# semicolonTransistor/rust-ray-tracing

Measured on AMD Instinct MI355X. Metric: Msamples/s (pixels×spp/s), 1920×1080·512spp·500 spheres; 1/2/4/8 GPU, higher is better.
Workload: dtype f32

## Files before the change

rust-ray-tracing_amd/csrc/rt_sweep.hpp:

```cpp
#pragma once
#include "rt_common.hpp"

namespace rt {

__device__ __forceinline__ uint32_t filter_group(const SphGroup<float>& cur, f2 K0, f2 K1, f2 K2, f2 K3, uint32_t& s0,
                                                 uint32_t& s1, f2* D = nullptr) {
    const f2 cx0 = {cur.v[0], cur.v[1]}, cy0 = {cur.v[2], cur.v[3]}, cz0 = {cur.v[4], cur.v[5]}, rr0 = {cur.v[6], cur.v[7]};
    const f2 cx1 = {cur.v[8], cur.v[9]}, cy1 = {cur.v[10], cur.v[11]}, cz1 = {cur.v[12], cur.v[13]}, rr1 = {cur.v[14], cur.v[15]};
    f2 a0, b0, a1, b1, r0, r1;
    asm volatile(
        "v_pk_fma_f32 %[a0], %[cz0], %[K0], %[K3] op_sel:[0,1,0] op_sel_hi:[1,1,0]\n\t"
        "v_pk_fma_f32 %[b0], %[cz0], %[K2], %[K3] op_sel:[0,0,1] op_sel_hi:[1,0,1]\n\t"
        "v_pk_fma_f32 %[a1], %[cz1], %[K0], %[K3] op_sel:[0,1,0] op_sel_hi:[1,1,0]\n\t"
        "v_pk_fma_f32 %[b1], %[cz1], %[K2], %[K3] op_sel:[0,0,1] op_sel_hi:[1,0,1]\n\t"
        "v_pk_fma_f32 %[a0], %[cx0], %[K0], %[a0] op_sel_hi:[1,0,1]\n\t"
        "v_pk_fma_f32 %[b0], %[cy0], %[K1], %[b0] op_sel:[0,1,0] op_sel_hi:[1,1,1]\n\t"
        "v_pk_fma_f32 %[a1], %[cx1], %[K0], %[a1] op_sel_hi:[1,0,1]\n\t"
        "v_pk_fma_f32 %[b1], %[cy1], %[K1], %[b1] op_sel:[0,1,0] op_sel_hi:[1,1,1]\n\t"
        "v_pk_fma_f32 %[b0], %[cx0], %[K1], %[b0] op_sel_hi:[1,0,1]\n\t"
        "v_pk_fma_f32 %[b1], %[cx1], %[K1], %[b1] op_sel_hi:[1,0,1]\n\t"
        "v_pk_fma_f32 %[r0], %[b0], %[b0], %[rr0] neg_lo:[1,0,0] neg_hi:[1,0,0]\n\t"
        "v_pk_fma_f32 %[r1], %[b1], %[b1], %[rr1] neg_lo:[1,0,0] neg_hi:[1,0,0]\n\t"
        "v_pk_fma_f32 %[r0], %[a0], %[a0], %[r0] neg_lo:[1,0,0] neg_hi:[1,0,0]\n\t"
        "v_pk_fma_f32 %[r1], %[a1], %[a1], %[r1] neg_lo:[1,0,0] neg_hi:[1,0,0]"
        : [a0] "=&v"(a0), [b0] "=&v"(b0), [a1] "=&v"(a1), [b1] "=&v"(b1), [r0] "=&v"(r0), [r1] "=&v"(r1)
        : [cx0] "s"(cx0), [cy0] "s"(cy0), [cz0] "s"(cz0), [rr0] "s"(rr0), [cx1] "s"(cx1), [cy1] "s"(cy1),
          [cz1] "s"(cz1), [rr1] "s"(rr1), [K0] "v"(K0), [K1] "v"(K1), [K2] "v"(K2), [K3] "v"(K3));
    s0 = __float_as_uint(r0.x) & __float_as_uint(r0.y);
    s1 = __float_as_uint(r1.x) & __float_as_uint(r1.y);
    if (D) { D[0] = r0; D[1] = r1; }
    return ~(s0 & s1);
}

__device__ __forceinline__ uint32_t cam_filter_group(const SphGroup<float>& cur, f2 K0, f2 K1) {
    const f2 ox0 = {cur.v[0], cur.v[1]}, oy0 = {cur.v[2], cur.v[3]}, oz0 = {cur.v[4], cur.v[5]}, sc0 = {cur.v[6], cur.v[7]};
    const f2 ox1 = {cur.v[8], cur.v[9]}, oy1 = {cur.v[10], cur.v[11]}, oz1 = {cur.v[12], cur.v[13]}, sc1 = {cur.v[14], cur.v[15]};
    f2 t0, t1;
    asm volatile(
        "v_pk_mul_f32 %[t0], %[ox0], %[K0] op_sel_hi:[1,0]\n\t"
        "v_pk_mul_f32 %[t1], %[ox1], %[K0] op_sel_hi:[1,0]\n\t"
        "v_pk_fma_f32 %[t0], %[oy0], %[K0], %[t0] op_sel:[0,1,0] op_sel_hi:[1,1,1]\n\t"
        "v_pk_fma_f32 %[t1], %[oy1], %[K0], %[t1] op_sel:[0,1,0] op_sel_hi:[1,1,1]\n\t"
        "v_pk_fma_f32 %[t0], %[oz0], %[K1], %[t0] op_sel_hi:[1,0,1]\n\t"
        "v_pk_fma_f32 %[t1], %[oz1], %[K1], %[t1] op_sel_hi:[1,0,1]\n\t"
        "v_pk_add_f32 %[t0], %[t0], %[sc0]\n\t"
        "v_pk_add_f32 %[t1], %[t1], %[sc1]"
        : [t0] "=&v"(t0), [t1] "=&v"(t1)
        : [ox0] "s"(ox0), [oy0] "s"(oy0), [oz0] "s"(oz0), [sc0] "s"(sc0), [ox1] "s"(ox1), [oy1] "s"(oy1),
          [oz1] "s"(oz1), [sc1] "s"(sc1), [K0] "v"(K0), [K1] "v"(K1));
    return (__float_as_uint(t0.x) | __float_as_uint(t0.y) | __float_as_uint(t1.x)) | __float_as_uint(t1.y);
}

__device__ __forceinline__ uint32_t box_pair(const float* v, f2 B0, f2 B1, f2 B2, f2 B3, f2 B4, float bt) {
    f2 ux, uy, uz, nx, ny, nz;
    const f2 cx = {v[0], v[1]}, cy = {v[2], v[3]}, cz = {v[4], v[5]}, hx = {v[6], v[7]}, hy = {v[8], v[9]},
             hz = {v[10], v[11]};
    asm volatile(
        "v_pk_fma_f32 %[ux], %[cx], %[B0], %[B2] op_sel_hi:[1,0,0]\n\t"
        "v_pk_fma_f32 %[uy], %[cy], %[B0], %[B2] op_sel:[0,1,1] op_sel_hi:[1,1,1]\n\t"
        "v_pk_fma_f32 %[uz], %[cz], %[B1], %[B1] op_sel:[0,0,1] op_sel_hi:[1,0,1]\n\t"
        "v_pk_fma_f32 %[nx], %[hx], %[B3], %[ux] op_sel_hi:[1,0,1] neg_lo:[0,1,0] neg_hi:[0,1,0]\n\t"
        "v_pk_fma_f32 %[ny], %[hy], %[B3], %[uy] op_sel:[0,1,0] op_sel_hi:[1,1,1] neg_lo:[0,1,0] neg_hi:[0,1,0]\n\t"
        "v_pk_fma_f32 %[nz], %[hz], %[B4], %[uz] op_sel_hi:[1,0,1] neg_lo:[0,1,0] neg_hi:[0,1,0]\n\t"
        "v_pk_fma_f32 %[ux], %[hx], %[B3], %[ux] op_sel_hi:[1,0,1]\n\t"
        "v_pk_fma_f32 %[uy], %[hy], %[B3], %[uy] op_sel:[0,1,0] op_sel_hi:[1,1,1]\n\t"
        "v_pk_fma_f32 %[uz], %[hz], %[B4], %[uz] op_sel_hi:[1,0,1]"
        : [ux] "=&v"(ux), [uy] "=&v"(uy), [uz] "=&v"(uz), [nx] "=&v"(nx), [ny] "=&v"(ny), [nz] "=&v"(nz)
        : [cx] "s"(cx), [cy] "s"(cy), [cz] "s"(cz), [hx] "s"(hx), [hy] "s"(hy), [hz] "s"(hz), [B0] "v"(B0),
          [B1] "v"(B1), [B2] "v"(B2), [B3] "v"(B3), [B4] "v"(B4));
    auto pass = [bt](float nx, float ny, float nz, float fx, float fy, float fz, auto bitc) -> uint32_t {
        constexpr uint32_t bit = decltype(bitc)::value;
        float tn, tf;
        unsigned long long m;
        uint32_t r;
        asm volatile(
            "v_max3_f32 %[tn], %[nx], %[ny], %[nz]\n\t"
            "v_min3_f32 %[tf], %[fx], %[fy], %[fz]\n\t"
            "v_max_f32 %[tn], 0, %[tn]\n\t"
            "v_min_f32 %[tf], %[tf], %[bt]\n\t"
            "v_cmp_nlt_f32_e64 %[m], %[tf], %[tn]\n\t"
            "s_cmp_lg_u64 %[m], 0\n\t"
            "s_cselect_b32 %[r], %[bit], 0"
            : [tn] "=&v"(tn), [tf] "=&v"(tf), [m] "=&s"(m), [r] "=s"(r)
            : [nx] "v"(nx), [ny] "v"(ny), [nz] "v"(nz), [fx] "v"(fx), [fy] "v"(fy), [fz] "v"(fz), [bt] "v"(bt),
              [bit] "n"(bit)
            : "scc");
        return r;
    };
    return __builtin_amdgcn_readfirstlane(pass(nx.x, ny.x, nz.x, ux.x, uy.x, uz.x, std::integral_constant<uint32_t, 1>{}) |
                                          pass(nx.y, ny.y, nz.y, ux.y, uy.y, uz.y, std::integral_constant<uint32_t, 2>{}));
}
__device__ __forceinline__ uint32_t box_mask(const BoxGroup& cur, f2 B0, f2 B1, f2 B2, f2 B3, f2 B4, float bt) {
    return box_pair(&cur.v[0], B0, B1, B2, B3, B4, bt) | (box_pair(&cur.v[12], B0, B1, B2, B3, B4, bt) << 2);
}
__device__ __forceinline__ uint32_t box_mask(const LBoxGroup& cur, f2 B0, f2 B1, f2 B2, f2 B3, f2 B4, float bt) {
    return box_pair(&cur.v[0], B0, B1, B2, B3, B4, bt) | (box_pair(&cur.v[12], B0, B1, B2, B3, B4, bt) << 2);
}

template <typename T> struct HitBest {
    T t = T(INFINITY);
    int i = -1;
    __device__ __forceinline__ T bt() const { return t; }
    __device__ __forceinline__ int bi() const { return i; }
    __device__ __forceinline__ void set(T r, uint32_t j) { t = r; i = (int)j; }
};
constexpr uint32_t kT001 = 0x3A83126Fu;
__device__ __forceinline__ uint64_t hit_key(float r, uint32_t j) {
    return ((uint64_t)(__float_as_uint(r) - kT001) << 32) | (uint64_t)~j;
}
template <> struct HitBest<float> {
    uint64_t k = (uint64_t)(0x7F800000u - kT001) << 32;
    __device__ __forceinline__ float bt() const { return __uint_as_float((uint32_t)(k >> 32) + kT001); }
    __device__ __forceinline__ int bi() const { return (int)~(uint32_t)k; }
    __device__ __forceinline__ void set(float r, uint32_t j) { k = hit_key(r, j); }
};
template <typename T, bool root2, bool SCALAR>
__device__ __forceinline__ void hit_update(T hb, T disc, uint32_t i, T a, T inv_a, HitBest<T>& bh) {
    if constexpr (SCALAR) {
        const T sd = sqrt(disc);
        T root = (-hb - sd) / a;
        if (!(root >= T(0.001) && root < T(INFINITY))) {
            root = (-hb + sd) / a;
            if (!(root >= T(0.001) && root < T(INFINITY))) return;
        }
        if (root < bh.bt() || (root == bh.bt() && (int)i < bh.bi())) bh.set(root, i);
        return;
    }
    const T sd = sqrt_len(disc);
    const T r1 = (-hb - sd) * inv_a;
    if constexpr (sizeof(T) == 4 && !root2) {
        const uint64_t key = hit_key(r1, i);
        bh.k = key < bh.k ? key : bh.k;
        return;
    }
    bool valid = r1 >= T(0.001) && r1 < T(INFINITY);
    T root = r1;
    if (root2 && !valid) {
        root = (-hb + sd) * inv_a;
        valid = root >= T(0.001) && root < T(INFINITY);
    }
    if constexpr (sizeof(T) == 4) {
        const uint64_t key = hit_key(root, i);
        const bool take = valid & (key < bh.k);
        bh.k = take ? key : bh.k;
    } else {
        const bool take = valid & ((root < bh.t) | ((root == bh.t) & ((int)i > bh.i)));
        bh.t = take ? root : bh.t;
        bh.i = take ? (int)i : bh.i;
    }
}

template <typename T, bool root2, bool SCALAR = false, bool CAMT = false, bool MEGA = false>
__device__ __forceinline__ int nearest_hit(const KParams<T>& p, const V3<T>& o, const V3<T>& d, T& t_out) {
    const T a = SCALAR ? len2(d) : pk_len2(d);
    const T inv_a = SCALAR ? T(0) : T(1.0) / a;
    HitBest<T> bh;
    KSTAT(CAMT ? 3 : 1);
    auto hit = [&](T hb, T disc, uint32_t i) { hit_update<T, root2, SCALAR>(hb, disc, i, a, inv_a, bh); };
    auto sbits = [](T x) -> uint32_t {
        if constexpr (sizeof(T) == 4) return __float_as_uint(x);
        else return (uint32_t)__double2hiint(x);
    };
    constexpr bool kBothRoots = root2 || SCALAR;
    auto is_cand = [](uint32_t m) -> bool { return (int32_t)m < 0; };
    auto cand_f = [&](T hb, T disc) -> bool { return kBothRoots ? disc >= T(0.0) : (disc >= T(0.0) && hb <= T(0.0)); };
    if constexpr (CAMT && !kBothRoots) {
        const auto& qa = *cold_args<T>();
        cptr<float> ff = (cptr<float>)__builtin_assume_aligned(qa.camf, 64);
        cptr<T> fe = (cptr<T>)__builtin_assume_aligned(qa.camsph, 64);
        const uint32_t ngf = qa.n_fgroups;
        const float fdx = (float)d.x, fdy = (float)d.y, fdz = (float)d.z;
        const float inv = 1.0f / sqrtf(__builtin_fmaf(fdz, fdz, __builtin_fmaf(fdy, fdy, fdx * fdx)));
        const f2 K0 = {fdx * inv, fdy * inv}, K1 = {fdz * inv, 0.0f};
        auto exact4 = [&](uint32_t g) {
            KSTAT(2);
            if constexpr (sizeof(T) == 4) {
                const SphGroup<T> cur = load_group(fe, g);
                const f2 dx = {d.x, d.x}, dy = {d.y, d.y}, dz = {d.z, d.z};
                const f2 na = {-a, -a};
                f2 hb[2], disc[2];
#pragma unroll
                for (uint32_t q = 0; q < 2; ++q) {
                    const T* v = &cur.v[8 * q];
                    const f2 ocx = {v[0], v[1]}, ocy = {v[2], v[3]}, ocz = {v[4], v[5]}, c = {v[6], v[7]};
                    hb[q] = fma2(ocz, dz, fma2(ocy, dy, ocx * dx));
                    disc[q] = fma2(hb[q], hb[q], na * c);
                }
                const uint32_t i0 = 4 * g;
                if (cand_f(hb[0].x, disc[0].x)) hit(hb[0].x, disc[0].x, i0);
                if (cand_f(hb[0].y, disc[0].y)) hit(hb[0].y, disc[0].y, i0 + 1);
                if (cand_f(hb[1].x, disc[1].x)) hit(hb[1].x, disc[1].x, i0 + 2);
                if (cand_f(hb[1].y, disc[1].y)) hit(hb[1].y, disc[1].y, i0 + 3);
            } else {
                const SphGroup<T> c0 = load_group(fe, 2 * g), c1 = load_group(fe, 2 * g + 1);
                T hb[4], disc[4];
#pragma unroll
                for (uint32_t j = 0; j < 4; ++j) {
                    const T* v = j < 2 ? &c0.v[4 * j] : &c1.v[4 * (j - 2)];
                    hb[j] = pk_dot(mk(v[0], v[1], v[2]), d);
                    disc[j] = fma(hb[j], hb[j], -a * v[3]);
                }
#pragma unroll
                for (uint32_t j = 0; j < 4; ++j)
                    if (cand_f(hb[j], disc[j])) hit(hb[j], disc[j], 4 * g + j);
            }
        };
        auto group = [&](const SphGroup<float>& cur, uint32_t g) {
            if (is_cand(cam_filter_group(cur, K0, K1))) exact4(g);
        };
        sphere_loop(ff, ngf, group);
    } else if constexpr (CAMT) {
        const auto& qa = *cold_args<T>();
        cptr<T> f = (cptr<T>)__builtin_assume_aligned(qa.camsph, 64);
        const uint32_t ng = qa.n_groups;
        if constexpr (sizeof(T) == 4) {
            const f2 dx = {d.x, d.x}, dy = {d.y, d.y}, dz = {d.z, d.z};
            const f2 na = {-a, -a};
            auto group = [&](const SphGroup<T>& cur, uint32_t g) {
                f2 hb[2], disc[2];
#pragma unroll
                for (uint32_t q = 0; q < 2; ++q) {
                    const T* v = &cur.v[8 * q];
                    const f2 ocx = {v[0], v[1]}, ocy = {v[2], v[3]}, ocz = {v[4], v[5]}, c = {v[6], v[7]};
                    if constexpr (SCALAR) {
                        hb[q] = (ocx * dx + ocy * dy) + ocz * dz;
                        disc[q] = hb[q] * hb[q] - (-na) * c;
                    } else {
                        hb[q] = fma2(ocz, dz, fma2(ocy, dy, ocx * dx));
                        disc[q] = fma2(hb[q], hb[q], na * c);
                    }
                }
                const uint32_t t = sbits(disc[0].x) & sbits(disc[0].y) & sbits(disc[1].x);
                const uint32_t acc = __builtin_amdgcn_bitop3_b32(t, sbits(disc[1].y), 0u, 0x3F);
                if (is_cand(acc)) {
                    KSTAT(2);
                    const uint32_t i0 = 4 * g;
                    if (cand_f(hb[0].x, disc[0].x)) hit(hb[0].x, disc[0].x, i0);
                    if (cand_f(hb[0].y, disc[0].y)) hit(hb[0].y, disc[0].y, i0 + 1);
                    if (cand_f(hb[1].x, disc[1].x)) hit(hb[1].x, disc[1].x, i0 + 2);
                    if (cand_f(hb[1].y, disc[1].y)) hit(hb[1].y, disc[1].y, i0 + 3);
                }
            };
            sphere_loop(f, ng, group);
        } else {
            auto group = [&](const SphGroup<T>& cur, uint32_t g) {
                T hb[2], disc[2];
#pragma unroll
                for (uint32_t j = 0; j < 2; ++j) {
                    const T* v = &cur.v[4 * j];
                    const V3<T> oc = mk(v[0], v[1], v[2]);
                    hb[j] = SCALAR ? dot(oc, d) : pk_dot(oc, d);
                    disc[j] = SCALAR ? hb[j] * hb[j] - a * v[3] : fma(hb[j], hb[j], -a * v[3]);
                }
                const uint32_t acc = __builtin_amdgcn_bitop3_b32(sbits(disc[0]), sbits(disc[1]), 0u, 0x3F);
                if (is_cand(acc)) {
                    KSTAT(2);
                    if (cand_f(hb[0], disc[0])) hit(hb[0], disc[0], 2 * g);
                    if (cand_f(hb[1], disc[1])) hit(hb[1], disc[1], 2 * g + 1);
                }
            };
            sphere_loop(f, ng, group);
        }
    } else {
        const auto& qa = *cold_args<T>();
        cptr<float> ff = (cptr<float>)__builtin_assume_aligned(qa.rfsph, 64);
        cptr<T> fe = (cptr<T>)__builtin_assume_aligned(qa.rsph, 64);
        auto sidx = [&](uint32_t g, cptr<float> ip) -> Q4 {
            if (ip != nullptr) {
                cptr<uint32_t> r = (cptr<uint32_t>)ip;
                return Q4{r[0], r[1], r[2], r[3]};
            }
            const auto& qi = *cold_args<T>();
            cptr<uint32_t> ri = (cptr<uint32_t>)__builtin_assume_aligned(qi.ridx, 16);
            return Q4{ri[4 * g], ri[4 * g + 1], ri[4 * g + 2], ri[4 * g + 3]};
        };
        const float fdx = (float)d.x, fdy = (float)d.y, fdz = (float)d.z;
        const float fox = (float)o.x, foy = (float)o.y, foz = (float)o.z;
        const float L = __builtin_fmaf(fdz, fdz, fdx * fdx);
        const float af = __builtin_fmaf(fdz, fdz, __builtin_fmaf(fdy, fdy, fdx * fdx));
        const float on = fabsf(fox) + fabsf(foy) + fabsf(foz);
        const float pm = qa.f_cmax + on;
        const float m = kFilterMargin * __builtin_fmaf(pm, pm, qa.f_r2max);
        const float sg = MEGA ? 1.0f : __builtin_amdgcn_rsqf(__builtin_fmaf(m, qa.f_ir2, 1.0f));
        const float s1 = __builtin_amdgcn_rsqf(L) * sg, s2 = __builtin_amdgcn_rsqf(L * af) * sg;
        float e1x = fdz * s1, e1z = -fdx * s1;
        float e2x = -(fdx * fdy) * s2, e2y = L * s2, e2z = -(fdy * fdz) * s2;
        float oe1 = __builtin_fmaf(foz, e1z, fox * e1x);
        float oe2 = __builtin_fmaf(foz, e2z, __builtin_fmaf(foy, e2y, fox * e2x));
        auto inv_ax = [](float v) -> float {
            return __builtin_amdgcn_rcpf(fabsf(v) >= 1e-20f ? v : copysignf(1e-20f, v));
        };
        float ix = inv_ax(fdx), iy = inv_ax(fdy), iz = inv_ax(fdz);
        const float kap = 1.0f + __builtin_fmaf(m, qa.f_hir2, pm * qa.f_isr);
        float Jx = fabsf(ix) * kap, Jy = fabsf(iy) * kap, Jz = fabsf(iz) * kap;
        float Ax = -(fox * ix), Ay = -(foy * iy), Az = -(foz * iz);
        if (!(L >= 1e-15f) || !(pm <= 1e15f)) {
            e1x = e1z = e2x = e2y = e2z = 0.0f;
            oe1 = oe2 = 0.0f;
            ix = iy = iz = Jx = Jy = Jz = Ax = Ay = Az = 0.0f;
        }
        const f2 K0 = {e1x, e1z}, K1 = {e2x, e2y}, K2 = {e2z, 0.0f}, K3 = {-oe1, -oe2};
        const f2 B0 = {ix, iy}, B1 = {iz, Az}, B2 = {Ax, Ay}, B3 = {Jx, Jy}, B4 = {Jz, 0.0f};
        auto btf = [&]() -> float {
            if constexpr (sizeof(T) == 4) return bh.bt();
            else return (float)bh.bt() * (1.0f + 0x1.0p-22f);
        };
        const f2 nixy = {-ix, -iy}, aixy = {fabsf(ix), fabsf(iy)};
        const float aiz = fabsf(iz);
        auto lmask = [&](const LBoxGroup& g) -> uint32_t {
            const auto& ql = *cold_args<T>();
            const f2 Sxy = {g.v[24], g.v[25]};
            const float Sz = g.v[26], Rg = g.v[27];
            f2 opxy;
            float opz;
            if constexpr (sizeof(T) == 4) {
                opxy = f2{o.x, o.y} - Sxy;
                opz = o.z - Sz;
            } else {
                opxy = f2{(float)(o.x - (double)Sxy.x), (float)(o.y - (double)Sxy.y)};
                opz = (float)(o.z - (double)Sz);
            }
            const float pmg = ((fabsf(opxy.x) + fabsf(opxy.y)) + fabsf(opz)) + Rg;
            const float kp = __builtin_fmaf(__builtin_fmaf(pmg, pmg, ql.l_r2max), ql.l_hir2,
                                            __builtin_fmaf(pmg, ql.l_isr, 1.0f));
            const f2 C1 = {iz, -(opz * iz)}, C2 = opxy * nixy;
            const f2 C3 = aixy * f2{kp, kp}, C4 = {aiz * kp, 0.0f};
            return box_mask(g, B0, C1, C2, C3, C4, btf());
        };
        auto exact4 = [&](uint32_t g, uint32_t pairs = sizeof(T) == 4 ? 3u : 15u, cptr<float> ip = nullptr) {
            KSTAT(0);
            if constexpr (sizeof(T) == 4) {
                const SphGroup<T> cur = load_group(fe, g);
                const f2 ox = {o.x, o.x}, oy = {o.y, o.y}, oz = {o.z, o.z};
                const f2 dx = {d.x, d.x}, dy = {d.y, d.y}, dz = {d.z, d.z};
                const f2 na = {-a, -a};
                const Q4 si = sidx(g, ip);
#pragma unroll
                for (uint32_t q = 0; q < 2; ++q) {
                    if (!((pairs >> q) & 1u)) continue;
                    f2 hb, disc;
                    const T* v = &cur.v[8 * q];
                    const f2 cx = {v[0], v[1]}, cy = {v[2], v[3]}, cz = {v[4], v[5]}, r2 = {v[6], v[7]};
                    const f2 ocx = ox - cx, ocy = oy - cy, ocz = oz - cz;
                    if constexpr (SCALAR) {
                        hb = (ocx * dx + ocy * dy) + ocz * dz;
                        const f2 c = ((ocx * ocx + ocy * ocy) + ocz * ocz) - r2;
                        disc = hb * hb - (-na) * c;
                    } else {
                        hb = fma2(ocz, dz, fma2(ocy, dy, ocx * dx));
                        const f2 c = fma2(ocz, ocz, fma2(ocy, ocy, ocx * ocx)) - r2;
                        disc = fma2(hb, hb, na * c);
                    }
                    if (cand_f(hb.x, disc.x)) hit(hb.x, disc.x, q ? si.z : si.x);
                    if (cand_f(hb.y, disc.y)) hit(hb.y, disc.y, q ? si.w : si.y);
                }
            } else {
                const SphGroup<T> c0 = load_group(fe, 2 * g), c1 = load_group(fe, 2 * g + 1);
                T hb[4], disc[4];
#pragma unroll
                for (uint32_t j = 0; j < 4; ++j) {
                    if (!((pairs >> j) & 1u)) continue;
                    const T* v = j < 2 ? &c0.v[4 * j] : &c1.v[4 * (j - 2)];
                    const V3<T> oc = mk(o.x - v[0], o.y - v[1], o.z - v[2]);
                    if constexpr (SCALAR) {
                        hb[j] = dot(oc, d);
                        disc[j] = hb[j] * hb[j] - a * (len2(oc) - v[3]);
                    } else {
                        hb[j] = pk_dot(oc, d);
                        const T c = pk_len2(oc) - v[3];
                        disc[j] = fma(hb[j], hb[j], -a * c);
                    }
                }
                const Q4 si = sidx(g, ip);
                const uint32_t sv[4] = {si.x, si.y, si.z, si.w};
#pragma unroll
                for (uint32_t j = 0; j < 4; ++j)
                    if (((pairs >> j) & 1u) && cand_f(hb[j], disc[j])) hit(hb[j], disc[j], sv[j]);
            }
        };
        auto exact4f = [&](const SphGroup<float>& cur, cptr<float> recp, uint32_t pairs) {
            KSTAT(0);
            if constexpr (sizeof(T) == 4) {
                cptr<uint32_t> xr = (cptr<uint32_t>)recp;
                uint32_t rec[8];
#pragma unroll
                for (int j = 0; j < 8; ++j) rec[j] = xr[(uint32_t)j];
                const f2 ox = {o.x, o.x}, oy = {o.y, o.y}, oz = {o.z, o.z};
                const f2 dx = {d.x, d.x}, dy = {d.y, d.y}, dz = {d.z, d.z};
                const f2 na = {-a, -a};
#pragma unroll
                for (uint32_t q = 0; q < 2; ++q) {
                    if (!((pairs >> q) & 1u)) continue;
                    f2 hb, disc;
                    const float* v = &cur.v[8 * q];
                    const f2 cx = {v[0], v[1]}, cy = {v[2], v[3]}, cz = {v[4], v[5]};
                    const f2 r2 = {__uint_as_float(rec[2 * q]), __uint_as_float(rec[2 * q + 1])};
                    const f2 ocx = ox - cx, ocy = oy - cy, ocz = oz - cz;
                    if constexpr (SCALAR) {
                        hb = (ocx * dx + ocy * dy) + ocz * dz;
                        const f2 c = ((ocx * ocx + ocy * ocy) + ocz * ocz) - r2;
                        disc = hb * hb - (-na) * c;
                    } else {
                        hb = fma2(ocz, dz, fma2(ocy, dy, ocx * dx));
                        const f2 c = fma2(ocz, ocz, fma2(ocy, ocy, ocx * ocx)) - r2;
                        disc = fma2(hb, hb, na * c);
                    }
                    if (cand_f(hb.x, disc.x)) hit(hb.x, disc.x, rec[4 + 2 * q]);
                    if (cand_f(hb.y, disc.y)) hit(hb.y, disc.y, rec[5 + 2 * q]);
                }
            }
        };
        const uint32_t nxg = qa.n_xg, ntop = qa.n_top;
        uint32_t n_box = 0, n_filt = 0, n_exact = 0;
        for (uint32_t g = 0; g < nxg; ++g) {
            const uint32_t pr = sizeof(T) == 4 ? (4u * g + 2u >= qa.n_xs ? 1u : 3u) : 15u;
            n_exact += pr == 1u ? 2u : 4u;
            exact4(g, pr);
        }
        cptr<float> ft = (cptr<float>)__builtin_assume_aligned(qa.ftop, 32);
        cptr<float> fs = (cptr<float>)__builtin_assume_aligned(qa.fsup, 32);
        const uint32_t nsg = (ntop + 3u) / 4u;
        auto walk_super = [&](uint32_t sup) {
            KSTAT(5);
            ++n_box;
            uint32_t mask;
            if constexpr (MEGA) {
                mask = lmask(load_lbox((cptr<float>)__builtin_assume_aligned(qa.lclb, 64), sup));
            }
            else mask = box_mask(load_box(ft, sup), B0, B1, B2, B3, B4, btf());
            while (mask != 0u) {
                const uint32_t kc = 4u * sup + (uint32_t)__builtin_ctz(mask);
                const uint32_t g0 = nxg + 4u * kc;
                mask &= mask - 1u;
                KSTAT(4);
                n_filt += 4u;
                f2 L0 = K0, L1 = K1, L2 = K2, L3 = K3;
                cptr<float> fg = ff;
                if constexpr (MEGA) {
                    const auto& ql = *cold_args<T>();
                    fg = (cptr<float>)__builtin_assume_aligned(ql.lfsph, 64) + 16u * nxg + 96u * kc;
                    const f2 Ckxy = {fg[64], fg[65]};
                    const float Ckz = fg[66];
                    const float Rc = fg[67], r2x = fg[72], ir2 = fg[73];
                    f2 opxy;
                    float opz;
                    if constexpr (sizeof(T) == 4) {
                        opxy = f2{o.x, o.y} - Ckxy;
                        opz = o.z - Ckz;
                    } else {
                        opxy = f2{(float)(o.x - (double)Ckxy.x), (float)(o.y - (double)Ckxy.y)};
                        opz = (float)(o.z - (double)Ckz);
                    }
                    const float opx = opxy.x, opy = opxy.y;
                    const float pmk = ((fabsf(opx) + fabsf(opy)) + fabsf(opz)) + Rc;
                    const float mk = kFilterMargin * __builtin_fmaf(pmk, pmk, r2x);
                    const float sgk = __builtin_amdgcn_rsqf(__builtin_fmaf(mk, ir2, 1.0f));
                    L0 = K0 * sgk; L1 = K1 * sgk; L2 = K2 * sgk;
                    const float oe1l = __builtin_fmaf(opz, L0.y, opx * L0.x);
                    const float oe2l = __builtin_fmaf(opz, L2.x, __builtin_fmaf(opy, L1.y, opx * L1.x));
                    L3 = f2{-oe1l, -oe2l};
                }
                constexpr bool kInl = sizeof(T) == 4 && !MEGA && !CAMT;
                const cptr<float> fgb = MEGA ? fg : ff + 16u * nxg + 96u * kc;
                sphere_loop(fgb, 4u, [&](const SphGroup<float>& cur, uint32_t g) {
                    uint32_t s0, s1;
                    f2 Dv[2];
                    const unsigned long long fpass = __ballot(is_cand(filter_group(cur, L0, L1, L2, L3, s0, s1, sizeof(T) == 8 ? Dv : nullptr)));
                    KSTAT(7, (uint32_t)__popcll(fpass));
                    if (fpass != 0ull) {
                        uint32_t pairs;
                        if constexpr (sizeof(T) == 4) {
                            pairs = (__ballot(!is_cand(s0)) != 0ull ? 1u : 0u) | (__ballot(!is_cand(s1)) != 0ull ? 2u : 0u);
                            n_exact += 2u * (uint32_t)__builtin_popcount(pairs);
                        } else {
                            auto ps = [](float D) -> bool { return (int32_t)__float_as_uint(D) >= 0; };
                            pairs = (__ballot(ps(Dv[0].x)) != 0ull ? 1u : 0u) | (__ballot(ps(Dv[0].y)) != 0ull ? 2u : 0u) |
                                    (__ballot(ps(Dv[1].x)) != 0ull ? 4u : 0u) | (__ballot(ps(Dv[1].y)) != 0ull ? 8u : 0u);
                            n_exact += (uint32_t)__builtin_popcount(pairs);
                        }
                        if constexpr (kInl) exact4f(cur, fgb + 64u + 8u * g, pairs);
                        else
                            exact4(g0 + g, pairs, fgb + 68u + 8u * g);
                    }
                });
            }
        };
        if constexpr (MEGA) {
            cptr<float> lm = (cptr<float>)__builtin_assume_aligned(qa.lmeg, 64);
            cptr<float> ls = (cptr<float>)__builtin_assume_aligned(qa.lsup, 64);
            const uint32_t ntg = qa.n_mg;
            auto walk_mega = [&](uint32_t nd) {
                ++n_box;
                uint32_t smask = lmask(load_lbox(ls, nd));
                if (4u * nd + 4u > ntop) smask &= (1u << (ntop - 4u * nd)) - 1u;
                while (smask != 0u) {
                    const uint32_t sup = 4u * nd + (uint32_t)__builtin_ctz(smask);
                    smask &= smask - 1u;
                    walk_super(sup);
                }
            };
            const uint32_t span = ntg <= 16u ? 16u : 8u;
            constexpr uint32_t kTest = 1;
            for (uint32_t t0 = 0; t0 < ntg; t0 += span) {
                const uint32_t nt = min(span, ntg - t0);
                const uint64_t valid = 4u * (t0 + nt) > nsg ? (1ull << (nsg - 4u * t0)) - 1ull : ~0ull;
                uint64_t T0 = 0, T1 = 0;
                if (span == 16u) {
                    const auto& qt = *cold_args<T>();
                    auto cell = [](float v, float lo, float inv, uint32_t n) -> uint32_t {
                        const float c = fminf(fmaxf((v - lo) * inv, 0.0f), (float)(n - 1u));
                        return __builtin_amdgcn_readfirstlane((uint32_t)c);
                    };
                    const uint32_t cx = cell((float)o.x, qt.mt_lo[0], qt.mt_inv, qt.mt_n[0]);
                    const uint32_t cy = cell((float)o.y, qt.mt_lo[1], qt.mt_inv, qt.mt_n[1]);
                    const uint32_t cz = cell((float)o.z, qt.mt_lo[2], qt.mt_inv, qt.mt_n[2]);
                    const uint32_t ci = 4u * (cx + qt.mt_n[0] * (cy + qt.mt_n[1] * cz));
                    cptr<uint64_t> tt = (cptr<uint64_t>)__builtin_assume_aligned(qt.mtiers, 32);
                    T0 = tt[ci] & valid;
                    T1 = tt[ci + 1u] & valid;
                }
                uint64_t tm = 0;
#pragma unroll 1
                for (uint32_t k = 0; k < 3u; ++k) {
                    if (k == kTest) {
                        const uint32_t ngg = span == 16u ? qa.n_gg : 0u;
                        if (ngg != 0u) {
                            uint32_t gm = 0;
                            n_box += ngg;
                            lbox_loop((cptr<float>)__builtin_assume_aligned(qa.lgig, 64), ngg,
                                      [&](const LBoxGroup& cur, uint32_t t) { gm |= lmask(cur) << (4u * t); });
                            gm &= (1u << nt) - 1u;
                            while (gm != 0u) {
                                const uint32_t gg = (uint32_t)__builtin_ctz(gm);
                                gm &= gm - 1u;
                                ++n_box;
                                tm |= (uint64_t)lmask(load_lbox(lm, gg)) << (4u * gg);
                            }
                        } else {
                            n_box += nt;
                            for (uint32_t t1 = 0; t1 < nt; t1 += 8u)
                                lbox_loop(lm + 32u * (t0 + t1), min(8u, nt - t1), [&](const LBoxGroup& cur, uint32_t t) {
                                    KSTAT(5);
                                    tm |= (uint64_t)lmask(cur) << (4u * (t1 + t));
                                });
                        }
                        tm &= valid;
                    }
                    uint64_t w = k == 0u ? (kTest == 0u ? tm & T0 : T0)
                                         : (k == 1u ? (kTest <= 1u ? tm & T1 : T1) & ~T0 : tm & ~T1);
                    while (w != 0ull) {
                        const uint32_t nd = 4u * t0 + (uint32_t)__builtin_ctzll(w);
                        w &= w - 1ull;
                        walk_mega(nd);
                    }
                }
            }
        } else {
            for (uint32_t t0 = 0; t0 < nsg; t0 += 8u) {
                uint32_t tmask = 0;
                n_box += min(8u, nsg - t0);
                box_loop(fs + kBoxFloats * t0, min(8u, nsg - t0), [&](const BoxGroup& cur, uint32_t t) {
                    KSTAT(5);
                    tmask |= box_mask(cur, B0, B1, B2, B3, B4, btf()) << (4u * t);
                });
                while (tmask != 0u) {
                    const uint32_t nd = 4u * t0 + (uint32_t)__builtin_ctz(tmask);
                    tmask &= tmask - 1u;
                    if (nd >= ntop) break;
                    walk_super(nd);
                }
            }
        }
        work_add(kWBox, n_box);
        work_add(kWFilt, n_filt);
        work_add(kWExact, n_exact);
    }
    t_out = bh.bt();
    return bh.bi();
}

}
```

Measured before the change: 38500.

## Defer per-sphere exact tests into per-lane candidate bitmask flush after filtering

For the f32 non-mega path, the per-group ballot and pair-wise exact test is replaced by accumulating sign bits of the filter results into per-lane bitmasks across all clusters of a supercluster. Each lane's candidate spheres are then tested individually in a flush loop, which loops while any lane has candidates left. This is meant to remove wave-divergent ballots and wasted exact tests on pairs where only some lanes pass, so exact work is compacted per lane. The cost is extra bit bookkeeping and index arithmetic, plus scattered loads per candidate. Lanes with few candidates idle while others finish the flush loop.

```diff
diff --git a/rust-ray-tracing_amd/csrc/rt_sweep.hpp b/rust-ray-tracing_amd/csrc/rt_sweep.hpp
--- a/rust-ray-tracing_amd/csrc/rt_sweep.hpp
+++ b/rust-ray-tracing_amd/csrc/rt_sweep.hpp
@@ -3,11 +3,10 @@
 
 namespace rt {
 
-__device__ __forceinline__ uint32_t filter_group(const SphGroup<float>& cur, f2 K0, f2 K1, f2 K2, f2 K3, uint32_t& s0,
-                                                 uint32_t& s1, f2* D = nullptr) {
+__device__ __forceinline__ void filter_group(const SphGroup<float>& cur, f2 K0, f2 K1, f2 K2, f2 K3, f2& r0, f2& r1) {
     const f2 cx0 = {cur.v[0], cur.v[1]}, cy0 = {cur.v[2], cur.v[3]}, cz0 = {cur.v[4], cur.v[5]}, rr0 = {cur.v[6], cur.v[7]};
     const f2 cx1 = {cur.v[8], cur.v[9]}, cy1 = {cur.v[10], cur.v[11]}, cz1 = {cur.v[12], cur.v[13]}, rr1 = {cur.v[14], cur.v[15]};
-    f2 a0, b0, a1, b1, r0, r1;
+    f2 a0, b0, a1, b1;
     asm volatile(
         "v_pk_fma_f32 %[a0], %[cz0], %[K0], %[K3] op_sel:[0,1,0] op_sel_hi:[1,1,0]\n\t"
         "v_pk_fma_f32 %[b0], %[cz0], %[K2], %[K3] op_sel:[0,0,1] op_sel_hi:[1,0,1]\n\t"
@@ -26,10 +25,6 @@
         : [a0] "=&v"(a0), [b0] "=&v"(b0), [a1] "=&v"(a1), [b1] "=&v"(b1), [r0] "=&v"(r0), [r1] "=&v"(r1)
         : [cx0] "s"(cx0), [cy0] "s"(cy0), [cz0] "s"(cz0), [rr0] "s"(rr0), [cx1] "s"(cx1), [cy1] "s"(cy1),
           [cz1] "s"(cz1), [rr1] "s"(rr1), [K0] "v"(K0), [K1] "v"(K1), [K2] "v"(K2), [K3] "v"(K3));
-    s0 = __float_as_uint(r0.x) & __float_as_uint(r0.y);
-    s1 = __float_as_uint(r1.x) & __float_as_uint(r1.y);
-    if (D) { D[0] = r0; D[1] = r1; }
-    return ~(s0 & s1);
 }
 
 __device__ __forceinline__ uint32_t cam_filter_group(const SphGroup<float>& cur, f2 K0, f2 K1) {
@@ -378,40 +373,39 @@
                     if (((pairs >> j) & 1u) && cand_f(hb[j], disc[j])) hit(hb[j], disc[j], sv[j]);
             }
         };
-        auto exact4f = [&](const SphGroup<float>& cur, cptr<float> recp, uint32_t pairs) {
-            KSTAT(0);
-            if constexpr (sizeof(T) == 4) {
-                cptr<uint32_t> xr = (cptr<uint32_t>)recp;
-                uint32_t rec[8];
-#pragma unroll
-                for (int j = 0; j < 8; ++j) rec[j] = xr[(uint32_t)j];
-                const f2 ox = {o.x, o.x}, oy = {o.y, o.y}, oz = {o.z, o.z};
-                const f2 dx = {d.x, d.x}, dy = {d.y, d.y}, dz = {d.z, d.z};
-                const f2 na = {-a, -a};
-#pragma unroll
-                for (uint32_t q = 0; q < 2; ++q) {
-                    if (!((pairs >> q) & 1u)) continue;
-                    f2 hb, disc;
-                    const float* v = &cur.v[8 * q];
-                    const f2 cx = {v[0], v[1]}, cy = {v[2], v[3]}, cz = {v[4], v[5]};
-                    const f2 r2 = {__uint_as_float(rec[2 * q]), __uint_as_float(rec[2 * q + 1])};
-                    const f2 ocx = ox - cx, ocy = oy - cy, ocz = oz - cz;
-                    if constexpr (SCALAR) {
-                        hb = (ocx * dx + ocy * dy) + ocz * dz;
-                        const f2 c = ((ocx * ocx + ocy * ocy) + ocz * ocz) - r2;
-                        disc = hb * hb - (-na) * c;
-                    } else {
-                        hb = fma2(ocz, dz, fma2(ocy, dy, ocx * dx));
-                        const f2 c = fma2(ocz, ocz, fma2(ocy, ocy, ocx * ocx)) - r2;
-                        disc = fma2(hb, hb, na * c);
-                    }
-                    if (cand_f(hb.x, disc.x)) hit(hb.x, disc.x, rec[4 + 2 * q]);
-                    if (cand_f(hb.y, disc.y)) hit(hb.y, disc.y, rec[5 + 2 * q]);
-                }
-            }
-        };
         const uint32_t nxg = qa.n_xg, ntop = qa.n_top;
         uint32_t n_box = 0, n_filt = 0, n_exact = 0;
+        auto flush = [&](cptr<float> blk, uint32_t cand) {
+            if constexpr (sizeof(T) == 4) {
+                while (__ballot(cand != 0u) != 0ull) {
+                    KSTAT(0);
+                    ++n_exact;
+                    if (cand != 0u) {
+                        const uint32_t b = (uint32_t)__builtin_ctz(cand);
+                        cand &= cand - 1u;
+                        const uint32_t s = (b & 15u) ^ 15u;
+                        const uint32_t cb = (b & 16u) * 6u;
+                        const uint32_t ic = cb + (((s & 14u) << 2) | (s & 1u));
+                        const uint32_t ir = cb + (((s & 12u) << 1) | (s & 3u));
+                        const float cx = blk[ic], cy = blk[ic + 2u], cz = blk[ic + 4u], r2 = blk[64u + ir];
+                        uint32_t si = ((cptr<uint32_t>)blk)[68u + ir];
+                        const float ocx = o.x - cx, ocy = o.y - cy, ocz = o.z - cz;
+                        float hb, disc;
+                        if constexpr (SCALAR) {
+                            hb = (ocx * d.x + ocy * d.y) + ocz * d.z;
+                            const float c = ((ocx * ocx + ocy * ocy) + ocz * ocz) - r2;
+                            disc = hb * hb - a * c;
+                        } else {
+                            hb = __builtin_fmaf(ocz, d.z, __builtin_fmaf(ocy, d.y, ocx * d.x));
+                            const float c = __builtin_fmaf(ocz, ocz, __builtin_fmaf(ocy, ocy, ocx * ocx)) - r2;
+                            disc = __builtin_fmaf(hb, hb, -a * c);
+                        }
+                        asm volatile("" : "+v"(si));
+                        if (cand_f(hb, disc)) hit(hb, disc, si);
+                    }
+                }
+            }
+        };
         for (uint32_t g = 0; g < nxg; ++g) {
             const uint32_t pr = sizeof(T) == 4 ? (4u * g + 2u >= qa.n_xs ? 1u : 3u) : 15u;
             n_exact += pr == 1u ? 2u : 4u;
@@ -428,8 +422,10 @@
                 mask = lmask(load_lbox((cptr<float>)__builtin_assume_aligned(qa.lclb, 64), sup));
             }
             else mask = box_mask(load_box(ft, sup), B0, B1, B2, B3, B4, btf());
+            uint32_t c01 = 0u, c23 = 0u;
             while (mask != 0u) {
-                const uint32_t kc = 4u * sup + (uint32_t)__builtin_ctz(mask);
+                const uint32_t kj = (uint32_t)__builtin_ctz(mask);
+                const uint32_t kc = 4u * sup + kj;
                 const uint32_t g0 = nxg + 4u * kc;
                 mask &= mask - 1u;
                 KSTAT(4);
@@ -462,10 +458,20 @@
                 }
                 constexpr bool kInl = sizeof(T) == 4 && !MEGA && !CAMT;
                 const cptr<float> fgb = MEGA ? fg : ff + 16u * nxg + 96u * kc;
+                uint32_t fm = 0xFFFFu;
                 sphere_loop(fgb, 4u, [&](const SphGroup<float>& cur, uint32_t g) {
-                    uint32_t s0, s1;
                     f2 Dv[2];
-                    const unsigned long long fpass = __ballot(is_cand(filter_group(cur, L0, L1, L2, L3, s0, s1, sizeof(T) == 8 ? Dv : nullptr)));
+                    filter_group(cur, L0, L1, L2, L3, Dv[0], Dv[1]);
+                    if constexpr (kInl) {
+                        fm = __builtin_amdgcn_alignbit(fm, __float_as_uint(Dv[0].x), 31u);
+                        fm = __builtin_amdgcn_alignbit(fm, __float_as_uint(Dv[0].y), 31u);
+                        fm = __builtin_amdgcn_alignbit(fm, __float_as_uint(Dv[1].x), 31u);
+                        fm = __builtin_amdgcn_alignbit(fm, __float_as_uint(Dv[1].y), 31u);
+                        return;
+                    }
+                    const uint32_t s0 = __float_as_uint(Dv[0].x) & __float_as_uint(Dv[0].y);
+                    const uint32_t s1 = __float_as_uint(Dv[1].x) & __float_as_uint(Dv[1].y);
+                    const unsigned long long fpass = __ballot(is_cand(~(s0 & s1)));
                     KSTAT(7, (uint32_t)__popcll(fpass));
                     if (fpass != 0ull) {
                         uint32_t pairs;
@@ -478,11 +484,19 @@
                                     (__ballot(ps(Dv[1].x)) != 0ull ? 4u : 0u) | (__ballot(ps(Dv[1].y)) != 0ull ? 8u : 0u);
                             n_exact += (uint32_t)__builtin_popcount(pairs);
                         }
-                        if constexpr (kInl) exact4f(cur, fgb + 64u + 8u * g, pairs);
-                        else
-                            exact4(g0 + g, pairs, fgb + 68u + 8u * g);
+                        exact4(g0 + g, pairs, fgb + 68u + 8u * g);
                     }
                 });
+                if constexpr (kInl) {
+                    if (kj < 2u) c01 |= ~fm << (16u * kj);
+                    else c23 |= ~fm << (16u * kj - 32u);
+                }
+            }
+            if constexpr (sizeof(T) == 4 && !MEGA) {
+                KSTAT(7, (uint32_t)__popcll(__ballot((c01 | c23) != 0u)));
+                const cptr<float> sb = ff + 16u * nxg + 384u * sup;
+                flush(sb, c01);
+                flush(sb + 192u, c23);
             }
         };
         if constexpr (MEGA) {
```

New measurement: 39360, median of 6. 1.02x the previous value.
